# openGemini/openGemini

Hardware: NVIDIA H100
Metric: decoded+aggregated rows/s (higher is better)
Workload: dtype f64

## Files before the change

### include/ogpu.h

```cpp
#ifndef OGPU_H
#define OGPU_H

#include <stddef.h>
#include <stdint.h>

#ifdef __cplusplus
extern "C" {
#endif

#define OG_API __attribute__((visibility("default")))

enum {
    OG_OK = 0,
    OG_EOF = 1,
    OG_E_INVAL = -1,
    OG_E_CUDA = -2,
    OG_E_NOMEM = -3,
    OG_E_UNSUPPORTED = -4,
    OG_E_CORRUPT = -5,
    OG_E_ABORTED = -6,
    OG_E_TYPE = -7,
    OG_E_STATE = -8
};

// ... 117 lines not shown
    uint64_t segments_scanned;
    uint64_t page_bytes;
    uint64_t dir_bytes;
    uint64_t out_bytes;
    double kernel_ms;
    double h2d_ms;
    double main_kernel_ms;
    uint32_t kernel_launches;
    int32_t path;
    int32_t il_state;
    int32_t per_series_cells_used;
    double il_build_ms;
    uint64_t il_bytes;
    uint64_t general_segments;
    double merge_ms;
} og_stats;

typedef struct og_shard og_shard;
typedef struct og_query og_query;

OG_API int og_init(int device_ordinal);
OG_API int og_device_count(void);
OG_API const char *og_strerror(int status);
OG_API const char *og_last_error(void);
OG_API const char *og_version(void);
OG_API int og_release_cached_memory(void);

typedef struct og_tssp og_tssp;
OG_API int og_tssp_parse(const uint8_t *file, uint64_t len, og_tssp **out);
OG_API int og_tssp_desc(const og_tssp *t, og_shard_desc *out);
// ... 90 lines not shown
```

### opengemini_b200/_lib.py

```python
import ctypes as C
import os

_HERE = os.path.dirname(os.path.abspath(__file__))
LIB_PATH = os.environ.get("OGPU_LIB") or os.path.join(_HERE, "libogpu.so")

OG_OK, OG_EOF = 0, 1
OG_E_INVAL, OG_E_CUDA, OG_E_NOMEM, OG_E_UNSUPPORTED, OG_E_CORRUPT, OG_E_ABORTED, OG_E_TYPE, OG_E_STATE = -1, -2, -3, -4, -5, -6, -7, -8
TYPE_INT, TYPE_FLOAT, TYPE_STRING, TYPE_BOOL = 1, 3, 4, 5
AGG_COUNT, AGG_SUM, AGG_MIN, AGG_MAX, AGG_FIRST, AGG_LAST = 1, 2, 3, 4, 5, 6
F_TERM, F_AND, F_OR = 0, 1, 2
OP_LT, OP_LTE, OP_GT, OP_GTE, OP_EQ, OP_NEQ = 0, 1, 2, 3, 4, 5
GROUP_ALL, GROUP_PER_SERIES, GROUP_MAP = 0, 1, 2
Q_STRICT_ORDER = 1
Q_NO_FUSED = 2
Q_NO_FAST = 4
Q_QUERY_GRID = 16
SYNTH_F_HI, SYNTH_F_LO, SYNTH_INT_WALK, SYNTH_BOOL = 0, 1, 2, 3
SHARD_DEVICE_DATA = 1
FILE_OUT_OF_ORDER = 1

u8p, u32p, u64p, i64p, i32p = C.POINTER(C.c_uint8), C.POINTER(C.c_uint32), C.POINTER(C.c_uint64), C.POINTER(C.c_int64), C.POINTER(C.c_int32)


class FilterItem(C.Structure):
# ... 34 lines not shown


class DenseCol(C.Structure):
    _fields_ = [("values", C.c_void_p), ("valid", C.c_void_p), ("times", C.c_void_p), ("type", C.c_int32), ("func", C.c_int32)]


class DenseView(C.Structure):
    _fields_ = [("n_groups", C.c_uint32), ("n_buckets", C.c_uint32), ("start", C.c_int64), ("interval", C.c_int64),
                ("n_cols", C.c_uint32), ("cols", C.POINTER(DenseCol)), ("stream", C.c_void_p)]


class Stats(C.Structure):
    _fields_ = [("rows_decoded", C.c_uint64), ("segments_scanned", C.c_uint64), ("page_bytes", C.c_uint64),
                ("dir_bytes", C.c_uint64), ("out_bytes", C.c_uint64), ("kernel_ms", C.c_double), ("h2d_ms", C.c_double), ("main_kernel_ms", C.c_double),
                ("kernel_launches", C.c_uint32), ("path", C.c_int32), ("il_state", C.c_int32), ("per_series_cells_used", C.c_int32),
                ("il_build_ms", C.c_double), ("il_bytes", C.c_uint64), ("general_segments", C.c_uint64), ("merge_ms", C.c_double)]


class SynthColumn(C.Structure):
    _fields_ = [("type", C.c_int32), ("dist", C.c_int32), ("null_permille", C.c_uint32)]


class SynthDesc(C.Structure):
    _fields_ = [("n_series", C.c_uint32), ("rows_per_series", C.c_uint32), ("rows_per_segment", C.c_uint32),
                ("t0", C.c_int64), ("dt", C.c_int64), ("seed", C.c_uint64), ("n_columns", C.c_uint32),
                ("columns", C.POINTER(SynthColumn)), ("series_base", C.c_uint32)]


class ShardLayout(C.Structure):
    _fields_ = [("data_len", C.c_uint64), ("n_series", C.c_uint32), ("n_segments", C.c_uint32), ("n_columns", C.c_uint32)]

# ... 93 lines not shown
```

### opengemini_b200/csrc/api.cu

```cuda
#include <algorithm>
#include <cstdarg>
#include <cstdio>
#include <cstring>
#include <numeric>

#include "agg_kernels.cuh"
#include "il_build.cuh"
#include "fused_multi.cuh"
#include "fused_cols.cuh"
#include "snappy_load.cuh"
#include <cub/device/device_scan.cuh>
#include <cub/device/device_radix_sort.cuh>
#include "internal.h"

namespace ogpu {

static thread_local char g_err[512] = "";
void set_error(const char *fmt, ...) {
    va_list ap; va_start(ap, fmt); vsnprintf(g_err, sizeof g_err, fmt, ap); va_end(ap);
}
int cuda_fail(cudaError_t e, const char *what, const char *file, int line) {
    set_error("CUDA error %d (%s) at %s:%d: %s", (int)e, cudaGetErrorString(e), file, line, what);
    return OG_E_CUDA;
}
// ... 151 lines not shown
    else CU(cudaSetDevice(g_device));
    return OG_OK;
}
}
static int need_device() { return ogpu::ensure_device(); }
extern "C" {

OG_API void og_shard_close(og_shard *s) {
    if (!s) return;
    if (s->owns_data && s->d_data) dev_free(s->d_data);
    dev_free(s->d_series_seg_begin); dev_free(s->d_seg_series); dev_free(s->d_seg_rows); dev_free(s->d_tmin); dev_free(s->d_tmax);
    dev_free(s->d_page_off); dev_free(s->d_page_len); dev_free(s->d_sids);
    if (s->h_seg_buf) cudaFreeHost(s->h_seg_buf);
    if (s->d_seg_buf) dev_free(s->d_seg_buf);
    for (auto &c : s->il) {
        dev_free(c.words); dev_free(c.grp_off); dev_free(c.grp_rows); dev_free(c.grp_col); dev_free(c.ok); dev_free(c.lane_seg); dev_free(c.lane_rows);
        dev_free(c.lane_series); dev_free(c.lane_t0); dev_free(c.lane_dt); dev_free(c.gen_list);
    }
    delete s;
}

}
namespace ogpu {
int check_desc(const og_shard_desc *d) {
    if (d->n_columns > 64 || (d->n_segments && (!d->seg_tmin || !d->seg_tmax || !d->time_page_off || !d->time_page_len)) || (d->n_series && !d->series_seg_begin)) { set_error("bad shard descriptor"); return OG_E_INVAL; }
    for (uint32_t s = 0; s < d->n_series; s++) if (d->series_seg_begin[s] > d->series_seg_begin[s + 1]) { set_error("series_seg_begin not monotone at %u", s); return OG_E_INVAL; }
    if (d->n_series && d->series_seg_begin[d->n_series] != d->n_segments) { set_error("series_seg_begin[n_series] != n_segments"); return OG_E_INVAL; }
    for (uint32_t c = 0; c < d->n_columns; c++)
        if (d->columns[c].type != OG_TYPE_INT && d->columns[c].type != OG_TYPE_FLOAT && d->columns[c].type != OG_TYPE_BOOL && d->columns[c].type != OG_TYPE_STRING) {
            set_error("column %u: unknown column type %d", c, d->columns[c].type); return OG_E_UNSUPPORTED;
        }
// ... 302 lines not shown
    ic.state = -1;
    if (s->n_segments == 0 || s->col_types[col] != OG_TYPE_FLOAT) return OG_OK;
    const uint32_t nseg = s->n_segments;
    uint32_t J = s->n_series ? s->h_series_seg_begin[1] - s->h_series_seg_begin[0] : 0;
    for (uint32_t i = 0; i < s->n_series && J; i++) if (s->h_series_seg_begin[i + 1] - s->h_series_seg_begin[i] != J) J = 0;
    const uint32_t n_super = J ? (s->n_series + OG_IL_SUPER - 1) / OG_IL_SUPER : 1;
    const uint64_t n_dom64 = J ? (uint64_t)n_super * J : 1;
    if (n_dom64 >= (1ull << 31)) return OG_OK;
    const uint32_t n_dom = (uint32_t)n_dom64;
    int rc;
    struct Ev { cudaEvent_t e = nullptr; Ev() { cudaEventCreate(&e); } ~Ev() { if (e) cudaEventDestroy(e); } } ev0, ev1;
    cudaEventRecord(ev0.e, st);
    TmpBufs tmp;
    IlScanOut so{};
    uint32_t *seg_words; uint64_t *keys2; uint32_t *vals2;
    if ((rc = dalloc(&ic.ok, (size_t)nseg))) return rc;
    so.ok = ic.ok;
    if ((rc = tmp.get(&seg_words, nseg)) || (rc = tmp.get(&so.seg_t0, nseg)) || (rc = tmp.get(&so.seg_dt, nseg)) || (rc = tmp.get(&so.keys, nseg)) ||
        (rc = tmp.get(&so.vals, nseg)) || (rc = tmp.get(&keys2, nseg)) || (rc = tmp.get(&vals2, nseg)) || (rc = tmp.get(&so.dom_cnt, n_dom))) return rc;
    so.seg_words = seg_words;
    if ((rc = tmp.get(&so.misaligned, 1))) return rc;
    CU(cudaMemsetAsync(so.dom_cnt, 0, (size_t)n_dom * 4, st));
    CU(cudaMemsetAsync(so.misaligned, 0, 4, st));
    DirP d = make_dir(s);
    k_il_scan<<<(nseg + 255) / 256, 256, 0, st>>>(d, col, s->col_types[col], J, so);
    CU(cudaGetLastError());
    int dbits = 1; while ((1ull << dbits) < n_dom64 + 1) dbits++;
    {
        size_t tb = 0;
        CU(cub::DeviceRadixSort::SortPairs(nullptr, tb, so.keys, keys2, so.vals, vals2, (int)nseg, 0, (int)OG_IL_WORD_BITS + dbits, st));
        void *dtmp; if ((rc = tmp.get((uint8_t **)&dtmp, tb))) return rc;
        CU(cub::DeviceRadixSort::SortPairs(dtmp, tb, so.keys, keys2, so.vals, vals2, (int)nseg, 0, (int)OG_IL_WORD_BITS + dbits, st));
    }
    std::vector<uint32_t> dom_cnt(n_dom); uint32_t misaligned = 1;
    CU(cudaMemcpyAsync(dom_cnt.data(), so.dom_cnt, (size_t)n_dom * 4, cudaMemcpyDeviceToHost, st));
    CU(cudaMemcpyAsync(&misaligned, so.misaligned, 4, cudaMemcpyDeviceToHost, st));
    CU(cudaStreamSynchronize(st));
    std::vector<uint32_t> elem_first(n_dom), grp_first(n_dom);
    uint64_t n_elig = 0, ng64 = 0;
    for (uint32_t i = 0; i < n_dom; i++) { elem_first[i] = (uint32_t)n_elig; grp_first[i] = (uint32_t)ng64; n_elig += dom_cnt[i]; ng64 += (dom_cnt[i] + 31) / 32; }
    const uint32_t n_gen = nseg - (uint32_t)n_elig;
    if (n_gen) {
        if ((rc = dalloc(&ic.gen_list, (size_t)n_gen))) return rc;
        CU(cudaMemcpyAsync(ic.gen_list, vals2 + n_elig, (size_t)n_gen * 4, cudaMemcpyDeviceToDevice, st));
        ic.gen_host.resize(n_gen);
        CU(cudaMemcpyAsync(ic.gen_host.data(), vals2 + n_elig, (size_t)n_gen * 4, cudaMemcpyDeviceToHost, st));
        CU(cudaStreamSynchronize(st));
    }
    if (n_elig == 0) return OG_OK;
    const uint32_t ng = (uint32_t)ng64;
    ic.n_groups = ng; ic.J = J; ic.aligned = J != 0 && misaligned == 0; ic.n_super = n_super; ic.cols_per_super = OG_IL_SUPER / 32 + 1;
    ic.super_grp_first.assign(n_super + 1, ng);
    for (uint32_t sp = 0; sp < n_super; sp++) ic.super_grp_first[sp] = grp_first[J ? sp * J : 0];
    uint32_t *d_elem_first, *d_grp_first;
    if ((rc = tmp.get(&d_elem_first, n_dom)) || (rc = tmp.get(&d_grp_first, n_dom))) return rc;
    CU(cudaMemcpyAsync(d_elem_first, elem_first.data(), (size_t)n_dom * 4, cudaMemcpyHostToDevice, st));
    CU(cudaMemcpyAsync(d_grp_first, grp_first.data(), (size_t)n_dom * 4, cudaMemcpyHostToDevice, st));
    const size_t n_slots = (size_t)ng * 32;
    if ((rc = dalloc(&ic.lane_seg, n_slots)) || (rc = dalloc(&ic.lane_rows, n_slots)) || (rc = dalloc(&ic.lane_series, n_slots)) ||
        (rc = dalloc(&ic.lane_t0, n_slots)) || (rc = dalloc(&ic.lane_dt, n_slots)) || (rc = dalloc(&ic.grp_col, (size_t)ng)) ||
        (rc = dalloc(&ic.grp_rows, (size_t)ng)) || (rc = dalloc(&ic.grp_off, (size_t)ng))) return rc;
    CU(cudaMemsetAsync(ic.lane_seg, 0xff, n_slots * 4, st));
    CU(cudaMemsetAsync(ic.lane_rows, 0, n_slots * 4, st));
    IlAssign as{};
    as.keys = keys2; as.segs = vals2; as.elem_first = d_elem_first; as.grp_first = d_grp_first;
    as.seg_words = seg_words; as.seg_t0 = so.seg_t0; as.seg_dt = so.seg_dt; as.ok = ic.ok;
    as.lane_seg = ic.lane_seg; as.lane_rows = ic.lane_rows; as.lane_series = ic.lane_series; as.grp_col = ic.grp_col; as.lane_t0 = ic.lane_t0; as.lane_dt = ic.lane_dt;
    as.n_elig = (uint32_t)n_elig; as.J = J; as.cols_per_super = ic.cols_per_super;
    k_il_assign<<<(unsigned)((n_elig + 255) / 256), 256, 0, st>>>(d, as);
    k_il_group_rows<<<(unsigned)((n_slots + 255) / 256), 256, 0, st>>>(ng, ic.lane_seg, seg_words, ic.grp_rows);
    CU(cudaGetLastError());
    std::vector<uint32_t> gw(ng); std::vector<uint64_t> go(ng);
    CU(cudaMemcpyAsync(gw.data(), ic.grp_rows, (size_t)ng * 4, cudaMemcpyDeviceToHost, st));
    CU(cudaStreamSynchronize(st));
    uint64_t total = 0;
    for (uint32_t g = 0; g < ng; g++) { go[g] = total; total += (uint64_t)gw[g] * 32; }
    size_t free_b = 0, total_b = 0;
    CU(dev_mem_info(&free_b, &total_b));
    size_t headroom = (size_t)8 << 30;
    if (const char *ov = getenv("OGPU_IL_HEADROOM_MB")) headroom = (size_t)atoll(ov) << 20;
    if (total * 4 + headroom > free_b || dev_malloc((void **)&ic.words, total * 4) != cudaSuccess) {
        cudaGetLastError(); ic.words = nullptr; ic.state = -2;
        return OG_OK;
    }
    CU(cudaMemcpyAsync(ic.grp_off, go.data(), (size_t)ng * 8, cudaMemcpyHostToDevice, st));
    k_il_repack<<<(unsigned)((n_slots + 127) / 128), 128, 0, st>>>(d, col, ic.ok, ic.lane_seg, ic.grp_off, ic.grp_rows, ng, ic.words);
    CU(cudaGetLastError());
    cudaEventRecord(ev1.e, st);
    CU(cudaStreamSynchronize(st));
    float ms = 0; cudaEventElapsedTime(&ms, ev0.e, ev1.e);
    ic.n_words = total; ic.build_ms = ms; ic.state = 1;
    return OG_OK;
}

int build_plan(og_query *q) {
    og_shard *s = q->sh;
    const QueryP &p = q->qp;
    cudaStream_t st = q->stream;
    int rc;
    Plan *pl = new Plan;
    memset((void *)pl, 0, sizeof *pl);
    q->plan = pl;
    size_t cells_dense = (size_t)q->n_groups * p.n_buckets;
    for (uint32_t c = 0; c < p.n_calls; c++) {
        bool sel = p.calls[c].func >= OG_AGG_MIN && !(p.multi && p.calls[c].func <= OG_AGG_MAX);
        if ((rc = dalloc(&q->dense[c].val, cells_dense))) return rc;
// ... 92 lines not shown
        }
    }
    if (pl->fold) {
        ch.gc_tail0 = ic->n_super * ic->cols_per_super; ch.gc_edge0 = 2 * ch.gc_tail0; ch.gc_col0 = 0;
        ch.gc_cols = ch.gc_edge0 + 3 * ((s->n_series + 31) / 32);
        const size_t n = (size_t)p.n_buckets * ch.gc_cols;
        for (uint32_t c = 0; c < p.n_calls; c++) {
            bool sel = p.calls[c].func >= OG_AGG_MIN;
            if ((rc = salloc(q, &ch.gcells[c].val, n))) return rc;
            if ((rc = salloc(q, &ch.gcells[c].ok, n))) return rc;
            if (sel && (rc = salloc(q, &ch.gcells[c].tim, n))) return rc;
        }
    }
    if (pl->fast) {
        pl->il.words = ic->words; pl->il.grp_off = ic->grp_off; pl->il.grp_rows = ic->grp_rows; pl->il.grp_col = ic->grp_col;
        pl->il.lane_seg = ic->lane_seg; pl->il.lane_rows = ic->lane_rows; pl->il.lane_series = ic->lane_series; pl->il.lane_t0 = ic->lane_t0; pl->il.lane_dt = ic->lane_dt;
        pl->fm = 0; pl->times = false;
        for (uint32_t c = 0; c < p.n_calls; c++) {
            pl->fm |= 1 << (p.calls[c].func - 1);
            if (p.calls[c].func >= OG_AGG_MIN && !(p.multi && p.calls[c].func <= OG_AGG_MAX)) pl->times = true;
        }
        pl->fm |= FM_COUNT;
        q->path_used = pl->fold ? 3 : 2;
    }
    if (!pl->fused && !pl->multi) {
        TileP &tp = pl->tp;
        tp.R = std::max<uint32_t>(1, s->max_seg_rows);
        size_t per_seg = (size_t)tp.R * (p.n_cols * 9 + 8 + 1);
        size_t fb = 0, tb = 0;
        CU(dev_mem_info(&fb, &tb));
        const size_t tile_budget = std::max<size_t>((size_t)96 << 20, std::min<size_t>(fb / 4, (size_t)12 << 30));
// ... 124 lines not shown
    q->cells_dirty = err[2] != 0;
    if (err[0]) { set_error("segment %d failed to decode (device code %d)", err[1], err[0]); return map_dev_err(err[0]); }
    float ms = 0; cudaEventElapsedTime(&ms, q->ev0, q->ev1);
    double main_ms = 0;
    for (uint32_t i = 0; i < chunks_run; i++) { float m = 0; cudaEventElapsedTime(&m, q->main_ev[2 * i], q->main_ev[2 * i + 1]); main_ms += m; }
    og_stats &stt = q->stats;
    uint64_t keep_pb = stt.page_bytes, keep_rows = stt.rows_decoded, keep_segs = stt.segments_scanned;
    memset(&stt, 0, sizeof stt);
    stt.kernel_ms = ms; stt.main_kernel_ms = main_ms; stt.kernel_launches = launches; stt.path = q->path_used;
    stt.page_bytes = keep_pb; stt.rows_decoded = keep_pb ? keep_rows : s->n_rows; stt.segments_scanned = keep_pb ? keep_segs : segs_scanned;
    stt.dir_bytes = (uint64_t)segs_scanned * 32;
    stt.out_bytes = 0;
    for (uint32_t c = 0; c < p.n_calls; c++) stt.out_bytes += cells_dense * (9 + (q->dense[c].tim ? 8 : 0));
    if (p.n_cols == 1 && p.col_type[0] == OG_TYPE_FLOAT && p.col_index[0] < (int)s->il.size()) {
        const og_shard::IlCol &ic = s->il[p.col_index[0]];
        stt.il_state = ic.state; stt.il_build_ms = ic.build_ms; stt.il_bytes = ic.n_words * 4;
        stt.general_segments = ic.state == 1 ? (uint64_t)ic.gen_host.size() : s->n_segments;
    }
    stt.per_series_cells_used = err[2] != 0;
    q->ran = true;
    return OG_OK;
}

OG_API int og_query_dense(og_query *q, og_dense_view *out) {
    if (!q || !out) return OG_E_INVAL;
    if (!q->ran) { set_error("og_query_dense before og_query_run"); return OG_E_STATE; }
    const QueryP &p = q->qp;
    out->n_groups = q->n_groups; out->n_buckets = p.n_buckets; out->start = q->desc.interval ? p.start : 0; out->interval = q->desc.interval ? p.interval : 0;
    out->n_cols = p.n_calls;
    for (uint32_t c = 0; c < p.n_calls; c++) {
        q->dense_cols[c].values = q->dense[c].val; q->dense_cols[c].valid = q->dense[c].ok; q->dense_cols[c].times = q->dense[c].tim;
// ... 273 lines not shown
```

### opengemini_b200/csrc/fused_il.cuh

```cuda
#pragma once
#include "agg_kernels.cuh"

namespace ogpu {

__device__ __forceinline__ uint32_t smem_u32(const void *p) { return (uint32_t)__cvta_generic_to_shared(p); }
__device__ __forceinline__ uint32_t opaque(uint32_t x) { asm volatile("mov.u32 %0, %0;" : "+r"(x)); return x; }
template <int OFF> __device__ __forceinline__ uint32_t lds32o(uint32_t a) { uint32_t v; asm volatile("ld.shared.u32 %0, [%1+%2];" : "=r"(v) : "r"(a), "n"(OFF)); return v; }
__device__ __forceinline__ void mbar_init(uint32_t bar, uint32_t count) { asm volatile("mbarrier.init.shared::cta.b64 [%0], %1;" ::"r"(bar), "r"(count) : "memory"); }
__device__ __forceinline__ void mbar_init_fence() { asm volatile("fence.mbarrier_init.release.cluster;\nfence.proxy.async.shared::cta;" ::: "memory"); }
__device__ __forceinline__ void mbar_expect_tx(uint32_t bar, uint32_t bytes) { asm volatile("mbarrier.arrive.expect_tx.shared::cta.b64 _, [%0], %1;" ::"r"(bar), "r"(bytes) : "memory"); }
__device__ __forceinline__ void bulk_g2s(uint32_t dst, const void *src, uint32_t bytes, uint32_t bar) {
    asm volatile("cp.async.bulk.shared::cluster.global.mbarrier::complete_tx::bytes [%0], [%1], %2, [%3];" ::"r"(dst), "l"(src), "r"(bytes), "r"(bar) : "memory");
}
__device__ __forceinline__ bool mbar_wait(uint32_t bar, uint32_t parity) {
#pragma unroll 1
    for (uint32_t i = 0; i < (1u << 16); i++) {
        uint32_t ok;
        asm volatile("{\n.reg .pred p;\nmbarrier.try_wait.parity.shared::cta.b64 p, [%1], %2;\nselp.u32 %0, 1, 0, p;\n}" : "=r"(ok) : "r"(bar), "r"(parity) : "memory");
        if (ok) return true;
    }
    return false;
}

enum { FM_COUNT = 1, FM_SUM = 2, FM_MIN = 4, FM_MAX = 8, FM_FIRST = 16, FM_LAST = 32 };
enum { SEG_GENERAL = 0, SEG_FAST = 1, SEG_RAWX = 2 };

#ifndef OG_FAST_THREADS
#define OG_FAST_THREADS 128
#endif
#ifndef OG_FAST_MAXREG
#define OG_FAST_MAXREG 80
#endif
#ifndef OG_IL_NW
#define OG_IL_NW 64u
#endif
#ifndef OG_IL_B
#define OG_IL_B 16u
#endif
#ifndef OG_IL_K
#define OG_IL_K 10u
#endif
#ifndef OG_IL_UNROLL
#define OG_IL_UNROLL 2
#endif
#define OG_IL_NB (OG_IL_NW / OG_IL_B)
#define OG_IL_ROWS (OG_IL_NW + 2u)
#define OG_IL_PAD_WORDS 6u
#define OG_IL_HDR 7u
#define OG_IL_RAW_HDR 6u
#define OG_IL_NONE 0xffffffffu
#define OG_IL_RAWFLAG 0x80000000u
#define OG_IL_LOOKBITS (77u * OG_IL_K + 29u + 13u + 64u + 64u)
static_assert(OG_IL_NW % OG_IL_B == 0 && (OG_IL_NW & (OG_IL_NW - 1)) == 0, "ring geometry");
static_assert(OG_IL_NW - OG_IL_B > (OG_IL_LOOKBITS + 31u) / 32u + 2u, "ring too small for the round length: the slowest lane could not proceed");

struct IlP {
    const uint32_t *words;
    const uint64_t *grp_off;
    const uint32_t *grp_rows;
    const uint32_t *grp_col;
    const uint32_t *lane_seg;
    const uint32_t *lane_rows;
    const uint32_t *lane_series;
    const int64_t *lane_t0;
    const uint64_t *lane_dt;
};

__device__ __forceinline__ uint64_t udiv_est(uint64_t a, uint64_t b, double inv_b) {
    const double qd = __ull2double_rn(a) * inv_b;
    if ((a >> 63) || !(qd < 1125899906842624.0)) return a / b;
    uint64_t q = (uint64_t)qd;
    uint64_t r = a - q * b;
    if ((int64_t)r < 0) { do { q--; r += b; } while ((int64_t)r < 0); }
    else while (r >= b) { q++; r -= b; }
    return q;
}

// ... 44 lines not shown
    const long long st_clk0 = clock64();
    long long st_wait = 0;
#endif
    const uint32_t lane = threadIdx.x & 31;
    const uint32_t wid = __reduce_max_sync(FULL, threadIdx.x >> 5);
    const uint32_t grp = grp_begin + blockIdx.x * WPB + wid;
    if (grp >= grp_end) return;
    const uint32_t rows_w = __reduce_max_sync(FULL, il.grp_rows[grp]);
    if (rows_w == 0) return;
    const size_t slot = (size_t)grp * 32 + lane;
    const uint32_t seg = il.lane_seg[slot];
    bool active = seg != OG_IL_NONE && seg >= ch.seg_begin && seg < ch.seg_end;
    if (!__any_sync(FULL, active)) return;
    const size_t e = 2 * (size_t)(seg - ch.seg_begin);

    uint32_t rows = 0, series = 0, r_lo = 0, r_hi = 0; bool rawx = false;
    int64_t t0 = 0, dt = 1; uint64_t dtu = 1; double inv_dt = 1.0;
    const double inv_iv = 1.0 / __ull2double_rn((uint64_t)q.interval);
    if (active) {
        const uint32_t rf = il.lane_rows[slot];
        rows = rf & ~OG_IL_RAWFLAG; rawx = (rf & OG_IL_RAWFLAG) != 0; series = il.lane_series[slot];
        t0 = il.lane_t0[slot]; dtu = il.lane_dt[slot]; dt = (int64_t)dtu;
        inv_dt = 1.0 / __ull2double_rn(dtu);
        r_lo = 0; r_hi = rows - 1;
        if (t0 < q.tmin) { uint64_t k = udiv_est((uint64_t)(q.tmin - t0) + dtu - 1, dtu, inv_dt); r_lo = k > rows ? rows : (uint32_t)k; }
        { int64_t t_last = t0 + (int64_t)(rows - 1) * dt; if (t_last > q.tmax) { if (q.tmax < t0) r_lo = rows; else r_hi = (uint32_t)udiv_est((uint64_t)(q.tmax - t0), dtu, inv_dt); } }
        if (r_lo > r_hi || r_lo >= rows) { *(uint2 *)(ch.edge_bucket + e) = make_uint2(OG_NO_BUCKET, OG_NO_BUCKET); active = false; }
    }
    if (!__any_sync(FULL, active)) return;

    const uint32_t win = smem_u32(s_win) + wid * (OG_IL_ROWS * 128);
    const uint32_t col = opaque(win + lane * 4);
    const uint32_t bar0 = smem_u32(s_bar) + wid * (NB * 8);
    if (lane == 0) {
#pragma unroll
        for (uint32_t i = 0; i < NB; i++) mbar_init(bar0 + i * 8, 1);
// ... 117 lines not shown
    };

    uint32_t qp = 0, sr = 0, kfast = 0, CM = 0, CE = 0, m = 64, tr = 0, bad = 0; uint64_t MASK = 0;
    bool done = !active;
    uint64_t val = 0;

#ifdef OG_IL_STATS
    long long st_w0 = clock64();
#endif
    if (issued_b && !mbar_wait(bar0, 0)) hung = 1; else ready_b = issued_b ? 1 : 0;
#ifdef OG_IL_STATS
    st_wait += clock64() - st_w0;
#endif
    if (active && !hung) {
        val = fetch64(col, 0); qp = 64;
        if (rawx) { MASK = ~0ull; kfast = 64; }
        else { CM = 0; CE = 1; }
    }

    bool skipping = r_lo > 0;
    stop = skipping ? r_lo : (rb < r_hi + 1 ? rb : r_hi + 1);
    n_ev = stop;
    if (!skipping) { fi = val; mn = mx = u2d(val); n_mn = n_mx = n_ev; }
    if (done) n_ev = 0xffffffffu;

    auto retire = [&]() { done = true; n_ev = 0xffffffffu; CM = 0; CE = 0; MASK = 0; kfast = 0; };
    auto advance = [&]() {
        bool fin = false;
        if (skipping) { skipping = false; sum = 0.0; }
        else {
            fin = stop > r_hi;
            sum = 0.0;
// ... 176 lines not shown
```

### opengemini_b200/csrc/il_build.cuh

```cuda
#pragma once
#include "fused_il.cuh"

namespace ogpu {

#define OG_IL_SUPER 4096u
#define OG_IL_WORD_BITS 24u

struct IlScanOut {
    uint8_t *ok;
    uint32_t *seg_words;
    int64_t *seg_t0;
    uint64_t *seg_dt;
    uint64_t *keys;
    uint32_t *vals;
    uint32_t *dom_cnt;
    uint32_t *misaligned;
};

__global__ void k_il_scan(DirP d, int col, int col_type, uint32_t J, IlScanOut o) {
    uint32_t seg = blockIdx.x * blockDim.x + threadIdx.x;
    if (seg >= d.n_segments) return;
    uint8_t c = SEG_GENERAL; uint32_t nw = 0; int64_t t0 = 0; uint64_t dt = 0;
    const uint32_t rows = d.seg_rows[seg];
    if (rows >= 2 && rows < (1u << 22) && col_type == OG_TYPE_FLOAT) {
        size_t pi = (size_t)col * d.n_segments + seg, ti = (size_t)d.n_columns * d.n_segments + seg;
        const uint8_t *p = d.data + d.page_off[pi], *t = d.data + d.page_off[ti];
        uint32_t len = d.page_len[pi], tlen = d.page_len[ti];
        TimeDesc td;
        if (len >= 16 && tlen >= 16 && __ldg(p) == 31 && __ldg(t) == 32 && (__ldg(t + 5) >> 4) == 1 && ld_be32(p + 1) == rows &&
            parse_time_page(t, tlen, td) == D_OK && td.kind == 0 && td.delta > 0 && td.delta < (1ull << 40)) {
            const int tag = __ldg(p + 5) >> 4;
            if (tag == 3 && __ldg(p + 6) == 0x10) {
                c = SEG_FAST; nw = (len - OG_IL_HDR + 3) / 4 + OG_IL_PAD_WORDS;
            } else if (tag == 0 && len == OG_IL_RAW_HDR + 8 * (size_t)rows) {
                c = SEG_RAWX; nw = 2 * rows + OG_IL_PAD_WORDS;
            }
            if (nw >= (1u << OG_IL_WORD_BITS)) { c = SEG_GENERAL; nw = 0; }
            t0 = td.t0; dt = td.delta;
        }
    }
    o.ok[seg] = c; o.seg_words[seg] = nw; o.seg_t0[seg] = t0; o.seg_dt[seg] = dt; o.vals[seg] = seg;
    const uint32_t series = d.seg_series[seg];
    if (J) {
        const uint32_t ref = d.series_seg_begin[series / OG_IL_SUPER * OG_IL_SUPER] + (seg - d.series_seg_begin[series]);
        if (d.seg_tmin[seg] != d.seg_tmin[ref] || d.seg_tmax[seg] != d.seg_tmax[ref]) *o.misaligned = 1;
    }
    if (c == SEG_GENERAL) { o.keys[seg] = ~0ull; return; }
    const uint32_t dom = J ? (series / OG_IL_SUPER) * J + (seg - d.series_seg_begin[series]) : 0u;
    o.keys[seg] = ((uint64_t)dom << OG_IL_WORD_BITS) | nw;
    atomicAdd(&o.dom_cnt[dom], 1u);
}

struct IlAssign {
    const uint64_t *keys; const uint32_t *segs;
    const uint32_t *elem_first, *grp_first;
    const uint32_t *seg_words; const int64_t *seg_t0; const uint64_t *seg_dt; const uint8_t *ok;
    uint32_t *lane_seg, *lane_rows, *lane_series, *grp_col; int64_t *lane_t0; uint64_t *lane_dt;
    uint32_t n_elig, J, cols_per_super;
};
__global__ void k_il_assign(DirP d, IlAssign a) {
    uint32_t i = blockIdx.x * blockDim.x + threadIdx.x;
    if (i >= a.n_elig) return;
    const uint32_t seg = a.segs[i], dom = (uint32_t)(a.keys[i] >> OG_IL_WORD_BITS);
    const uint32_t rank = i - a.elem_first[dom], g = a.grp_first[dom] + rank / 32;
    const size_t slot = (size_t)g * 32 + (rank & 31);
    a.lane_seg[slot] = seg;
    a.lane_rows[slot] = d.seg_rows[seg] | (a.ok[seg] == SEG_RAWX ? OG_IL_RAWFLAG : 0u);
    a.lane_series[slot] = d.seg_series[seg];
    a.lane_t0[slot] = a.seg_t0[seg]; a.lane_dt[slot] = a.seg_dt[seg];
    if ((rank & 31) == 0) a.grp_col[g] = (a.J ? dom / a.J : 0u) * a.cols_per_super + rank / 32;
}

__global__ void k_il_group_rows(uint32_t n_groups, const uint32_t *lane_seg, const uint32_t *seg_words, uint32_t *grp_rows) {
    uint32_t g = (blockIdx.x * blockDim.x + threadIdx.x) >> 5, lane = threadIdx.x & 31;
    if (g >= n_groups) return;
    uint32_t seg = lane_seg[(size_t)g * 32 + lane];
    uint32_t w = seg != OG_IL_NONE ? seg_words[seg] : 0;
#pragma unroll
    for (int o = 16; o; o >>= 1) w = max(w, __shfl_xor_sync(0xffffffffu, w, o));
    if (lane == 0) grp_rows[g] = (w + OG_IL_B - 1) / OG_IL_B * OG_IL_B;
}

__global__ void k_il_repack(DirP d, int col, const uint8_t *ok, const uint32_t *lane_seg, const uint64_t *grp_off, const uint32_t *grp_rows,
                            uint32_t n_groups, uint32_t *il) {
    uint32_t g = (blockIdx.x * blockDim.x + threadIdx.x) >> 5, lane = threadIdx.x & 31;
    if (g >= n_groups) return;
    const uint32_t nw = grp_rows[g];
    if (nw == 0) return;
    const uint32_t seg = lane_seg[(size_t)g * 32 + lane];
    const bool live = seg != OG_IL_NONE;
    const bool raw = live && ok[seg] == SEG_RAWX;
    const uint32_t *base = nullptr; uint32_t sh = 0, own_words = 0;
    if (live) {
        size_t pi = (size_t)col * d.n_segments + seg;
        const uint8_t *s = d.data + d.page_off[pi] + (raw ? OG_IL_RAW_HDR : OG_IL_HDR);
        base = (const uint32_t *)((uintptr_t)s & ~(uintptr_t)3);
        sh = (uint32_t)((uintptr_t)s & 3);
        own_words = raw ? 2 * d.seg_rows[seg] : (d.page_len[pi] - OG_IL_HDR + 3) / 4 + OG_IL_PAD_WORDS;
    }
    uint32_t *out = il + grp_off[g] + lane;
    uint32_t a = live ? __ldg(base) : 0;
    if (!raw) {
        const uint32_t sel = sh == 0 ? 0x0123u : sh == 1 ? 0x1234u : sh == 2 ? 0x2345u : 0x3456u;
        for (uint32_t w = 0; w < nw; w++) {
            uint32_t v = 0;
            if (w < own_words) {
                uint32_t b = __ldg(base + w + 1);
                v = __byte_perm(a, b, sel);
                a = b;
            }
            out[(size_t)w * 32] = v;
        }
    } else {
        const uint32_t sel = sh == 0 ? 0x3210u : sh == 1 ? 0x4321u : sh == 2 ? 0x5432u : 0x6543u;
        uint32_t plo = 0, phi = 0;
        for (uint32_t w = 0; w < nw; w += 2) {
            uint32_t hi = 0, lo = 0;
            if (w < own_words) {
                uint32_t b = __ldg(base + w + 1), c = __ldg(base + w + 2);
                const uint32_t vlo = __byte_perm(a, b, sel), vhi = __byte_perm(b, c, sel);
                a = c;
                hi = vhi ^ phi; lo = vlo ^ plo; phi = vhi; plo = vlo;
            }
            out[(size_t)w * 32] = hi;
            if (w + 1 < nw) out[(size_t)(w + 1) * 32] = lo;
        }
    }
}

}
```

### opengemini_b200/csrc/internal.h

```cpp
#pragma once
#include <cuda_runtime.h>

#include <cstdint>
#include <string>
#include <mutex>
#include <vector>

#include "../../include/ogpu.h"

#define OG_MAX_CALLS 8
#define OG_MAX_FILTER 16
#define OG_MAX_COLS 8

namespace ogpu {

void set_error(const char *fmt, ...);
int cuda_fail(cudaError_t e, const char *what, const char *file, int line);
int ensure_device();

inline cudaError_t dev_malloc(void **p, size_t bytes) { return cudaMallocAsync(p, bytes ? bytes : 1, (cudaStream_t)0); }
inline void dev_free(void *p) { if (p) cudaFreeAsync(p, (cudaStream_t)0); }
cudaError_t dev_mem_info(size_t *free_b, size_t *total_b);
#define CU(call) do { cudaError_t e__ = (call); if (e__ != cudaSuccess) return ::ogpu::cuda_fail(e__, #call, __FILE__, __LINE__); } while (0)

// ... 16 lines not shown
    std::vector<uint64_t> sids;
    std::vector<int32_t> col_types;
    std::vector<std::string> col_names;
    std::vector<uint32_t> h_series_seg_begin;
    uint32_t *d_series_seg_begin = nullptr;
    uint32_t *d_seg_series = nullptr;
    uint32_t *d_seg_rows = nullptr;
    int64_t *d_tmin = nullptr, *d_tmax = nullptr;
    uint64_t *d_page_off = nullptr;
    uint32_t *d_page_len = nullptr;
    uint64_t *d_sids = nullptr;
    void *h_seg_buf = nullptr; size_t h_seg_buf_bytes = 0;
    void *d_seg_buf = nullptr; size_t d_seg_buf_bytes = 0;
    std::vector<og_colval_view> seg_views;
    struct IlCol { int state = 0;
                   uint32_t *words = nullptr; uint64_t *grp_off = nullptr; uint32_t *grp_rows = nullptr, *grp_col = nullptr; uint8_t *ok = nullptr;
                   uint32_t *lane_seg = nullptr, *lane_rows = nullptr, *lane_series = nullptr; int64_t *lane_t0 = nullptr; uint64_t *lane_dt = nullptr;
                   uint32_t *gen_list = nullptr; std::vector<uint32_t> gen_host;
                   uint32_t n_groups = 0, J = 0;
                   bool aligned = false;
                   uint32_t n_super = 1, cols_per_super = 0; std::vector<uint32_t> super_grp_first;
                   uint64_t n_words = 0; double build_ms = 0; };
    std::vector<IlCol> il;
    std::mutex il_mu;
};

namespace ogpu {

struct CallP { int32_t func, col_slot, type, out_type; };
struct FilterP { int32_t kind, col_slot, op, type, const_is_float; double fval; int64_t ival; };

struct Tri { uint64_t *val; int64_t *tim; uint8_t *ok; };

struct QueryP {
    int64_t tmin, tmax, start, interval;
    uint32_t n_buckets, n_calls, n_filter, n_cols;
    int32_t multi;
// ... 43 lines not shown
```

Measured before the change: 378.9 billion.

## Repack float segments as fixed-width XOR-delta windows in interleaved layout

At build time the IL scan now measures, per float segment, the leading-zero and meaningful-bit window of XOR deltas between consecutive values. When this fixed-width packing is smaller than the Gorilla-style stream, or the page is raw, the segment is repacked into packed m-bit deltas. The fused kernel then decodes these lanes with a fixed mask instead of the variable control-bit path. The intent is to cut bytes read and branchy decode per row, at the cost of a heavier build-time scan and repack plus a new per-lane window array.

```diff
diff --git a/include/ogpu.h b/include/ogpu.h
--- a/include/ogpu.h
+++ b/include/ogpu.h
@@ -155,6 +155,7 @@
     uint64_t il_bytes;
     uint64_t general_segments;
     double merge_ms;
+    uint64_t il_packed_segments;
 } og_stats;
 
 typedef struct og_shard og_shard;
diff --git a/opengemini_b200/_lib.py b/opengemini_b200/_lib.py
--- a/opengemini_b200/_lib.py
+++ b/opengemini_b200/_lib.py
@@ -72,7 +72,8 @@
     _fields_ = [("rows_decoded", C.c_uint64), ("segments_scanned", C.c_uint64), ("page_bytes", C.c_uint64),
                 ("dir_bytes", C.c_uint64), ("out_bytes", C.c_uint64), ("kernel_ms", C.c_double), ("h2d_ms", C.c_double), ("main_kernel_ms", C.c_double),
                 ("kernel_launches", C.c_uint32), ("path", C.c_int32), ("il_state", C.c_int32), ("per_series_cells_used", C.c_int32),
-                ("il_build_ms", C.c_double), ("il_bytes", C.c_uint64), ("general_segments", C.c_uint64), ("merge_ms", C.c_double)]
+                ("il_build_ms", C.c_double), ("il_bytes", C.c_uint64), ("general_segments", C.c_uint64), ("merge_ms", C.c_double),
+                ("il_packed_segments", C.c_uint64)]
 
 
 class SynthColumn(C.Structure):
diff --git a/opengemini_b200/csrc/api.cu b/opengemini_b200/csrc/api.cu
--- a/opengemini_b200/csrc/api.cu
+++ b/opengemini_b200/csrc/api.cu
@@ -189,7 +189,7 @@
     if (s->h_seg_buf) cudaFreeHost(s->h_seg_buf);
     if (s->d_seg_buf) dev_free(s->d_seg_buf);
     for (auto &c : s->il) {
-        dev_free(c.words); dev_free(c.grp_off); dev_free(c.grp_rows); dev_free(c.grp_col); dev_free(c.ok); dev_free(c.lane_seg); dev_free(c.lane_rows);
+        dev_free(c.words); dev_free(c.grp_off); dev_free(c.grp_rows); dev_free(c.grp_col); dev_free(c.lane_seg); dev_free(c.lane_rows); dev_free(c.lane_win);
         dev_free(c.lane_series); dev_free(c.lane_t0); dev_free(c.lane_dt); dev_free(c.gen_list);
     }
     delete s;
@@ -522,14 +522,14 @@
     TmpBufs tmp;
     IlScanOut so{};
     uint32_t *seg_words; uint64_t *keys2; uint32_t *vals2;
-    if ((rc = dalloc(&ic.ok, (size_t)nseg))) return rc;
-    so.ok = ic.ok;
-    if ((rc = tmp.get(&seg_words, nseg)) || (rc = tmp.get(&so.seg_t0, nseg)) || (rc = tmp.get(&so.seg_dt, nseg)) || (rc = tmp.get(&so.keys, nseg)) ||
+    if ((rc = tmp.get(&so.seg_win, nseg)) || (rc = tmp.get(&so.n_packed, 1)) ||
+        (rc = tmp.get(&seg_words, nseg)) || (rc = tmp.get(&so.seg_t0, nseg)) || (rc = tmp.get(&so.seg_dt, nseg)) || (rc = tmp.get(&so.keys, nseg)) ||
         (rc = tmp.get(&so.vals, nseg)) || (rc = tmp.get(&keys2, nseg)) || (rc = tmp.get(&vals2, nseg)) || (rc = tmp.get(&so.dom_cnt, n_dom))) return rc;
     so.seg_words = seg_words;
     if ((rc = tmp.get(&so.misaligned, 1))) return rc;
     CU(cudaMemsetAsync(so.dom_cnt, 0, (size_t)n_dom * 4, st));
     CU(cudaMemsetAsync(so.misaligned, 0, 4, st));
+    CU(cudaMemsetAsync(so.n_packed, 0, 8, st));
     DirP d = make_dir(s);
     k_il_scan<<<(nseg + 255) / 256, 256, 0, st>>>(d, col, s->col_types[col], J, so);
     CU(cudaGetLastError());
@@ -540,9 +540,10 @@
         void *dtmp; if ((rc = tmp.get((uint8_t **)&dtmp, tb))) return rc;
         CU(cub::DeviceRadixSort::SortPairs(dtmp, tb, so.keys, keys2, so.vals, vals2, (int)nseg, 0, (int)OG_IL_WORD_BITS + dbits, st));
     }
-    std::vector<uint32_t> dom_cnt(n_dom); uint32_t misaligned = 1;
+    std::vector<uint32_t> dom_cnt(n_dom); uint32_t misaligned = 1; unsigned long long n_packed = 0;
     CU(cudaMemcpyAsync(dom_cnt.data(), so.dom_cnt, (size_t)n_dom * 4, cudaMemcpyDeviceToHost, st));
     CU(cudaMemcpyAsync(&misaligned, so.misaligned, 4, cudaMemcpyDeviceToHost, st));
+    CU(cudaMemcpyAsync(&n_packed, so.n_packed, 8, cudaMemcpyDeviceToHost, st));
     CU(cudaStreamSynchronize(st));
     std::vector<uint32_t> elem_first(n_dom), grp_first(n_dom);
     uint64_t n_elig = 0, ng64 = 0;
@@ -565,15 +566,16 @@
     CU(cudaMemcpyAsync(d_elem_first, elem_first.data(), (size_t)n_dom * 4, cudaMemcpyHostToDevice, st));
     CU(cudaMemcpyAsync(d_grp_first, grp_first.data(), (size_t)n_dom * 4, cudaMemcpyHostToDevice, st));
     const size_t n_slots = (size_t)ng * 32;
-    if ((rc = dalloc(&ic.lane_seg, n_slots)) || (rc = dalloc(&ic.lane_rows, n_slots)) || (rc = dalloc(&ic.lane_series, n_slots)) ||
+    if ((rc = dalloc(&ic.lane_seg, n_slots)) || (rc = dalloc(&ic.lane_rows, n_slots)) || (rc = dalloc(&ic.lane_win, n_slots)) || (rc = dalloc(&ic.lane_series, n_slots)) ||
         (rc = dalloc(&ic.lane_t0, n_slots)) || (rc = dalloc(&ic.lane_dt, n_slots)) || (rc = dalloc(&ic.grp_col, (size_t)ng)) ||
         (rc = dalloc(&ic.grp_rows, (size_t)ng)) || (rc = dalloc(&ic.grp_off, (size_t)ng))) return rc;
     CU(cudaMemsetAsync(ic.lane_seg, 0xff, n_slots * 4, st));
     CU(cudaMemsetAsync(ic.lane_rows, 0, n_slots * 4, st));
+    CU(cudaMemsetAsync(ic.lane_win, 0, n_slots * 2, st));
     IlAssign as{};
     as.keys = keys2; as.segs = vals2; as.elem_first = d_elem_first; as.grp_first = d_grp_first;
-    as.seg_words = seg_words; as.seg_t0 = so.seg_t0; as.seg_dt = so.seg_dt; as.ok = ic.ok;
-    as.lane_seg = ic.lane_seg; as.lane_rows = ic.lane_rows; as.lane_series = ic.lane_series; as.grp_col = ic.grp_col; as.lane_t0 = ic.lane_t0; as.lane_dt = ic.lane_dt;
+    as.seg_words = seg_words; as.seg_t0 = so.seg_t0; as.seg_dt = so.seg_dt; as.seg_win = so.seg_win;
+    as.lane_seg = ic.lane_seg; as.lane_rows = ic.lane_rows; as.lane_series = ic.lane_series; as.grp_col = ic.grp_col; as.lane_win = ic.lane_win; as.lane_t0 = ic.lane_t0; as.lane_dt = ic.lane_dt;
     as.n_elig = (uint32_t)n_elig; as.J = J; as.cols_per_super = ic.cols_per_super;
     k_il_assign<<<(unsigned)((n_elig + 255) / 256), 256, 0, st>>>(d, as);
     k_il_group_rows<<<(unsigned)((n_slots + 255) / 256), 256, 0, st>>>(ng, ic.lane_seg, seg_words, ic.grp_rows);
@@ -592,12 +594,12 @@
         return OG_OK;
     }
     CU(cudaMemcpyAsync(ic.grp_off, go.data(), (size_t)ng * 8, cudaMemcpyHostToDevice, st));
-    k_il_repack<<<(unsigned)((n_slots + 127) / 128), 128, 0, st>>>(d, col, ic.ok, ic.lane_seg, ic.grp_off, ic.grp_rows, ng, ic.words);
+    k_il_repack<<<(unsigned)((n_slots + 127) / 128), 128, 0, st>>>(d, col, ic.lane_seg, ic.lane_win, ic.grp_off, ic.grp_rows, ng, ic.words);
     CU(cudaGetLastError());
     cudaEventRecord(ev1.e, st);
     CU(cudaStreamSynchronize(st));
     float ms = 0; cudaEventElapsedTime(&ms, ev0.e, ev1.e);
-    ic.n_words = total; ic.build_ms = ms; ic.state = 1;
+    ic.n_words = total; ic.n_packed = n_packed; ic.build_ms = ms; ic.state = 1;
     return OG_OK;
 }
 
@@ -720,7 +722,7 @@
     }
     if (pl->fast) {
         pl->il.words = ic->words; pl->il.grp_off = ic->grp_off; pl->il.grp_rows = ic->grp_rows; pl->il.grp_col = ic->grp_col;
-        pl->il.lane_seg = ic->lane_seg; pl->il.lane_rows = ic->lane_rows; pl->il.lane_series = ic->lane_series; pl->il.lane_t0 = ic->lane_t0; pl->il.lane_dt = ic->lane_dt;
+        pl->il.lane_seg = ic->lane_seg; pl->il.lane_rows = ic->lane_rows; pl->il.lane_win = ic->lane_win; pl->il.lane_series = ic->lane_series; pl->il.lane_t0 = ic->lane_t0; pl->il.lane_dt = ic->lane_dt;
         pl->fm = 0; pl->times = false;
         for (uint32_t c = 0; c < p.n_calls; c++) {
             pl->fm |= 1 << (p.calls[c].func - 1);
@@ -875,7 +877,7 @@
     for (uint32_t c = 0; c < p.n_calls; c++) stt.out_bytes += cells_dense * (9 + (q->dense[c].tim ? 8 : 0));
     if (p.n_cols == 1 && p.col_type[0] == OG_TYPE_FLOAT && p.col_index[0] < (int)s->il.size()) {
         const og_shard::IlCol &ic = s->il[p.col_index[0]];
-        stt.il_state = ic.state; stt.il_build_ms = ic.build_ms; stt.il_bytes = ic.n_words * 4;
+        stt.il_state = ic.state; stt.il_build_ms = ic.build_ms; stt.il_bytes = ic.n_words * 4; stt.il_packed_segments = ic.state == 1 ? ic.n_packed : 0;
         stt.general_segments = ic.state == 1 ? (uint64_t)ic.gen_host.size() : s->n_segments;
     }
     stt.per_series_cells_used = err[2] != 0;
diff --git a/opengemini_b200/csrc/fused_il.cuh b/opengemini_b200/csrc/fused_il.cuh
--- a/opengemini_b200/csrc/fused_il.cuh
+++ b/opengemini_b200/csrc/fused_il.cuh
@@ -23,7 +23,7 @@
 }
 
 enum { FM_COUNT = 1, FM_SUM = 2, FM_MIN = 4, FM_MAX = 8, FM_FIRST = 16, FM_LAST = 32 };
-enum { SEG_GENERAL = 0, SEG_FAST = 1, SEG_RAWX = 2 };
+enum { SEG_GENERAL = 0, SEG_FAST = 1, SEG_PACKED = 2 };
 
 #ifndef OG_FAST_THREADS
 #define OG_FAST_THREADS 128
@@ -49,8 +49,9 @@
 #define OG_IL_HDR 7u
 #define OG_IL_RAW_HDR 6u
 #define OG_IL_NONE 0xffffffffu
-#define OG_IL_RAWFLAG 0x80000000u
+#define OG_IL_PACKED 0x8000u
 #define OG_IL_LOOKBITS (77u * OG_IL_K + 29u + 13u + 64u + 64u)
+static_assert(OG_IL_K >= 2, "packed lanes: K*64 + 63 + 128 <= OG_IL_LOOKBITS needs K >= 2");
 static_assert(OG_IL_NW % OG_IL_B == 0 && (OG_IL_NW & (OG_IL_NW - 1)) == 0, "ring geometry");
 static_assert(OG_IL_NW - OG_IL_B > (OG_IL_LOOKBITS + 31u) / 32u + 2u, "ring too small for the round length: the slowest lane could not proceed");
 
@@ -61,6 +62,7 @@
     const uint32_t *grp_col;
     const uint32_t *lane_seg;
     const uint32_t *lane_rows;
+    const uint16_t *lane_win;
     const uint32_t *lane_series;
     const int64_t *lane_t0;
     const uint64_t *lane_dt;
@@ -135,12 +137,11 @@
     if (!__any_sync(FULL, active)) return;
     const size_t e = 2 * (size_t)(seg - ch.seg_begin);
 
-    uint32_t rows = 0, series = 0, r_lo = 0, r_hi = 0; bool rawx = false;
+    uint32_t rows = 0, series = 0, r_lo = 0, r_hi = 0, lwin = 0;
     int64_t t0 = 0, dt = 1; uint64_t dtu = 1; double inv_dt = 1.0;
     const double inv_iv = 1.0 / __ull2double_rn((uint64_t)q.interval);
     if (active) {
-        const uint32_t rf = il.lane_rows[slot];
-        rows = rf & ~OG_IL_RAWFLAG; rawx = (rf & OG_IL_RAWFLAG) != 0; series = il.lane_series[slot];
+        rows = il.lane_rows[slot]; lwin = il.lane_win[slot]; series = il.lane_series[slot];
         t0 = il.lane_t0[slot]; dtu = il.lane_dt[slot]; dt = (int64_t)dtu;
         inv_dt = 1.0 / __ull2double_rn(dtu);
         r_lo = 0; r_hi = rows - 1;
@@ -288,8 +289,11 @@
 #endif
     if (active && !hung) {
         val = fetch64(col, 0); qp = 64;
-        if (rawx) { MASK = ~0ull; kfast = 64; }
-        else { CM = 0; CE = 1; }
+        if (lwin & OG_IL_PACKED) {
+            const uint32_t lead = (lwin >> 8) & 63u, mw = lwin & 127u;
+            qp = 64 - lead; kfast = mw;
+            MASK = mw ? (~0ull >> (64 - mw)) << (64 - lead - mw) : 0ull;
+        } else { CM = 0; CE = 1; }
     }
 
     bool skipping = r_lo > 0;
diff --git a/opengemini_b200/csrc/il_build.cuh b/opengemini_b200/csrc/il_build.cuh
--- a/opengemini_b200/csrc/il_build.cuh
+++ b/opengemini_b200/csrc/il_build.cuh
@@ -7,8 +7,9 @@
 #define OG_IL_WORD_BITS 24u
 
 struct IlScanOut {
-    uint8_t *ok;
     uint32_t *seg_words;
+    uint16_t *seg_win;
+    unsigned long long *n_packed;
     int64_t *seg_t0;
     uint64_t *seg_dt;
     uint64_t *keys;
@@ -17,10 +18,27 @@
     uint32_t *misaligned;
 };
 
+__device__ inline bool il_delta_window(const uint8_t *page, uint32_t len, uint32_t rows, uint32_t m_stop, uint32_t &lead, uint32_t &m) {
+    ColIter it;
+    it.init(page, len, OG_TYPE_FLOAT, rows);
+    uint64_t prev = 0, acc = 0;
+    if (it.err != D_OK || !it.next(prev)) return false;
+    for (uint32_t r = 1; r < rows && it.err == D_OK; r++) {
+        uint64_t v = 0;
+        if (!it.next(v)) return false;
+        acc |= v ^ prev; prev = v;
+        if ((r & 31) == 0 && m_stop < 64 && acc && 64 - __clzll((long long)acc) - (__ffsll((long long)acc) - 1) >= (int)m_stop) return false;
+    }
+    if (it.err != D_OK) return false;
+    lead = acc ? (uint32_t)__clzll((long long)acc) : 0u;
+    m = acc ? 64u - lead - (uint32_t)(__ffsll((long long)acc) - 1) : 0u;
+    return true;
+}
+
 __global__ void k_il_scan(DirP d, int col, int col_type, uint32_t J, IlScanOut o) {
     uint32_t seg = blockIdx.x * blockDim.x + threadIdx.x;
     if (seg >= d.n_segments) return;
-    uint8_t c = SEG_GENERAL; uint32_t nw = 0; int64_t t0 = 0; uint64_t dt = 0;
+    uint8_t c = SEG_GENERAL; uint32_t nw = 0; int64_t t0 = 0; uint64_t dt = 0; uint16_t win = 0;
     const uint32_t rows = d.seg_rows[seg];
     if (rows >= 2 && rows < (1u << 22) && col_type == OG_TYPE_FLOAT) {
         size_t pi = (size_t)col * d.n_segments + seg, ti = (size_t)d.n_columns * d.n_segments + seg;
@@ -33,13 +51,27 @@
             if (tag == 3 && __ldg(p + 6) == 0x10) {
                 c = SEG_FAST; nw = (len - OG_IL_HDR + 3) / 4 + OG_IL_PAD_WORDS;
             } else if (tag == 0 && len == OG_IL_RAW_HDR + 8 * (size_t)rows) {
-                c = SEG_RAWX; nw = 2 * rows + OG_IL_PAD_WORDS;
+                c = SEG_PACKED; nw = 2 * rows + OG_IL_PAD_WORDS; win = OG_IL_PACKED | 64u;
             }
-            if (nw >= (1u << OG_IL_WORD_BITS)) { c = SEG_GENERAL; nw = 0; }
+            uint32_t m_stop = 64, lead, m;
+            if (c == SEG_FAST) {
+                const uint32_t T = nw > 2 + OG_IL_PAD_WORDS ? nw - 2 - OG_IL_PAD_WORDS : 0;
+                const uint64_t ms = T ? (32ull * (T - 1)) / (rows - 1) + 1 : 0;
+                m_stop = ms < 64 ? (uint32_t)ms : 64u;
+            }
+            if (c != SEG_GENERAL && il_delta_window(p, len, rows, m_stop, lead, m)) {
+                const uint32_t pw = 2u + (uint32_t)(((uint64_t)(rows - 1) * m + 31) / 32) + OG_IL_PAD_WORDS;
+                if (c == SEG_PACKED || pw < nw) { c = SEG_PACKED; nw = pw; win = (uint16_t)(OG_IL_PACKED | lead << 8 | m); }
+            }
+            if (nw >= (1u << OG_IL_WORD_BITS)) { c = SEG_GENERAL; nw = 0; win = 0; }
             t0 = td.t0; dt = td.delta;
         }
     }
-    o.ok[seg] = c; o.seg_words[seg] = nw; o.seg_t0[seg] = t0; o.seg_dt[seg] = dt; o.vals[seg] = seg;
+    o.seg_words[seg] = nw; o.seg_win[seg] = win; o.seg_t0[seg] = t0; o.seg_dt[seg] = dt; o.vals[seg] = seg;
+    {
+        const unsigned am = __activemask(), pm = __ballot_sync(am, c == SEG_PACKED);
+        if (pm && (threadIdx.x & 31) == (unsigned)(__ffs(am) - 1)) atomicAdd(o.n_packed, (unsigned long long)__popc(pm));
+    }
     const uint32_t series = d.seg_series[seg];
     if (J) {
         const uint32_t ref = d.series_seg_begin[series / OG_IL_SUPER * OG_IL_SUPER] + (seg - d.series_seg_begin[series]);
@@ -54,8 +86,8 @@
 struct IlAssign {
     const uint64_t *keys; const uint32_t *segs;
     const uint32_t *elem_first, *grp_first;
-    const uint32_t *seg_words; const int64_t *seg_t0; const uint64_t *seg_dt; const uint8_t *ok;
-    uint32_t *lane_seg, *lane_rows, *lane_series, *grp_col; int64_t *lane_t0; uint64_t *lane_dt;
+    const uint32_t *seg_words; const int64_t *seg_t0; const uint64_t *seg_dt; const uint16_t *seg_win;
+    uint32_t *lane_seg, *lane_rows, *lane_series, *grp_col; uint16_t *lane_win; int64_t *lane_t0; uint64_t *lane_dt;
     uint32_t n_elig, J, cols_per_super;
 };
 __global__ void k_il_assign(DirP d, IlAssign a) {
@@ -65,7 +97,8 @@
     const uint32_t rank = i - a.elem_first[dom], g = a.grp_first[dom] + rank / 32;
     const size_t slot = (size_t)g * 32 + (rank & 31);
     a.lane_seg[slot] = seg;
-    a.lane_rows[slot] = d.seg_rows[seg] | (a.ok[seg] == SEG_RAWX ? OG_IL_RAWFLAG : 0u);
+    a.lane_rows[slot] = d.seg_rows[seg];
+    a.lane_win[slot] = a.seg_win[seg];
     a.lane_series[slot] = d.seg_series[seg];
     a.lane_t0[slot] = a.seg_t0[seg]; a.lane_dt[slot] = a.seg_dt[seg];
     if ((rank & 31) == 0) a.grp_col[g] = (a.J ? dom / a.J : 0u) * a.cols_per_super + rank / 32;
@@ -81,50 +114,62 @@
     if (lane == 0) grp_rows[g] = (w + OG_IL_B - 1) / OG_IL_B * OG_IL_B;
 }
 
-__global__ void k_il_repack(DirP d, int col, const uint8_t *ok, const uint32_t *lane_seg, const uint64_t *grp_off, const uint32_t *grp_rows,
+__global__ void k_il_repack(DirP d, int col, const uint32_t *lane_seg, const uint16_t *lane_win, const uint64_t *grp_off, const uint32_t *grp_rows,
                             uint32_t n_groups, uint32_t *il) {
     uint32_t g = (blockIdx.x * blockDim.x + threadIdx.x) >> 5, lane = threadIdx.x & 31;
     if (g >= n_groups) return;
     const uint32_t nw = grp_rows[g];
     if (nw == 0) return;
-    const uint32_t seg = lane_seg[(size_t)g * 32 + lane];
+    const size_t slot = (size_t)g * 32 + lane;
+    const uint32_t seg = lane_seg[slot];
     const bool live = seg != OG_IL_NONE;
-    const bool raw = live && ok[seg] == SEG_RAWX;
-    const uint32_t *base = nullptr; uint32_t sh = 0, own_words = 0;
+    const uint32_t win = live ? lane_win[slot] : 0u;
+    const bool packed = (win & OG_IL_PACKED) != 0;
+    const uint32_t *base = nullptr; uint32_t sh = 0, own_words = 0, a = 0, sel = 0;
+    ColIter it;
+    uint64_t prev = 0, pend = 0, acc = 0; uint32_t pbits = 0, nb = 0, left = 0, mw = 0, tr = 0;
     if (live) {
-        size_t pi = (size_t)col * d.n_segments + seg;
-        const uint8_t *s = d.data + d.page_off[pi] + (raw ? OG_IL_RAW_HDR : OG_IL_HDR);
-        base = (const uint32_t *)((uintptr_t)s & ~(uintptr_t)3);
-        sh = (uint32_t)((uintptr_t)s & 3);
-        own_words = raw ? 2 * d.seg_rows[seg] : (d.page_len[pi] - OG_IL_HDR + 3) / 4 + OG_IL_PAD_WORDS;
+        const size_t pi = (size_t)col * d.n_segments + seg;
+        const uint8_t *page = d.data + d.page_off[pi];
+        if (packed) {
+            it.init(page, d.page_len[pi], OG_TYPE_FLOAT, d.seg_rows[seg]);
+            it.next(prev);
+            pend = prev; pbits = 64;
+            mw = win & 127u;
+            tr = mw ? 64u - ((win >> 8) & 63u) - mw : 0u;
+            left = mw ? d.seg_rows[seg] - 1 : 0u;
+        } else {
+            const uint8_t *s = page + OG_IL_HDR;
+            base = (const uint32_t *)((uintptr_t)s & ~(uintptr_t)3);
+            sh = (uint32_t)((uintptr_t)s & 3);
+            own_words = (d.page_len[pi] - OG_IL_HDR + 3) / 4 + OG_IL_PAD_WORDS;
+            a = __ldg(base);
+            sel = sh == 0 ? 0x0123u : sh == 1 ? 0x1234u : sh == 2 ? 0x2345u : 0x3456u;
+        }
     }
     uint32_t *out = il + grp_off[g] + lane;
-    uint32_t a = live ? __ldg(base) : 0;
-    if (!raw) {
-        const uint32_t sel = sh == 0 ? 0x0123u : sh == 1 ? 0x1234u : sh == 2 ? 0x2345u : 0x3456u;
-        for (uint32_t w = 0; w < nw; w++) {
-            uint32_t v = 0;
-            if (w < own_words) {
-                uint32_t b = __ldg(base + w + 1);
-                v = __byte_perm(a, b, sel);
-                a = b;
+    for (uint32_t w = 0; w < nw; w++) {
+        uint32_t v = 0;
+        if (packed) {
+            while (nb < 32) {
+                if (pbits == 0) {
+                    if (left == 0) break;
+                    uint64_t x = 0;
+                    it.next(x);
+                    pend = (x ^ prev) >> tr; prev = x; pbits = mw; left--;
+                }
+                const uint32_t k = pbits < 32 ? pbits : 32;
+                acc |= ((pend >> (pbits - k)) & (~0ull >> (64 - k))) << (64 - nb - k);
+                nb += k; pbits -= k;
             }
-            out[(size_t)w * 32] = v;
+            v = (uint32_t)(acc >> 32);
+            acc <<= 32; nb = nb > 32 ? nb - 32 : 0;
+        } else if (w < own_words) {
+            const uint32_t b = __ldg(base + w + 1);
+            v = __byte_perm(a, b, sel);
+            a = b;
         }
-    } else {
-        const uint32_t sel = sh == 0 ? 0x3210u : sh == 1 ? 0x4321u : sh == 2 ? 0x5432u : 0x6543u;
-        uint32_t plo = 0, phi = 0;
-        for (uint32_t w = 0; w < nw; w += 2) {
-            uint32_t hi = 0, lo = 0;
-            if (w < own_words) {
-                uint32_t b = __ldg(base + w + 1), c = __ldg(base + w + 2);
-                const uint32_t vlo = __byte_perm(a, b, sel), vhi = __byte_perm(b, c, sel);
-                a = c;
-                hi = vhi ^ phi; lo = vlo ^ plo; phi = vhi; plo = vlo;
-            }
-            out[(size_t)w * 32] = hi;
-            if (w + 1 < nw) out[(size_t)(w + 1) * 32] = lo;
-        }
+        out[(size_t)w * 32] = v;
     }
 }
 
diff --git a/opengemini_b200/csrc/internal.h b/opengemini_b200/csrc/internal.h
--- a/opengemini_b200/csrc/internal.h
+++ b/opengemini_b200/csrc/internal.h
@@ -54,13 +54,13 @@
     void *d_seg_buf = nullptr; size_t d_seg_buf_bytes = 0;
     std::vector<og_colval_view> seg_views;
     struct IlCol { int state = 0;
-                   uint32_t *words = nullptr; uint64_t *grp_off = nullptr; uint32_t *grp_rows = nullptr, *grp_col = nullptr; uint8_t *ok = nullptr;
-                   uint32_t *lane_seg = nullptr, *lane_rows = nullptr, *lane_series = nullptr; int64_t *lane_t0 = nullptr; uint64_t *lane_dt = nullptr;
+                   uint32_t *words = nullptr; uint64_t *grp_off = nullptr; uint32_t *grp_rows = nullptr, *grp_col = nullptr;
+                   uint32_t *lane_seg = nullptr, *lane_rows = nullptr, *lane_series = nullptr; uint16_t *lane_win = nullptr; int64_t *lane_t0 = nullptr; uint64_t *lane_dt = nullptr;
                    uint32_t *gen_list = nullptr; std::vector<uint32_t> gen_host;
                    uint32_t n_groups = 0, J = 0;
                    bool aligned = false;
                    uint32_t n_super = 1, cols_per_super = 0; std::vector<uint32_t> super_grp_first;
-                   uint64_t n_words = 0; double build_ms = 0; };
+                   uint64_t n_words = 0, n_packed = 0;  double build_ms = 0; };
     std::vector<IlCol> il;
     std::mutex il_mu;
 };
```

Measured after the change: 408.3 billion (median of 6 runs). +7.8%, better.
